# jibanCat/gp_dla_detection

Hardware: NVIDIA B200
Metric: qso_spectra_per_sec_10k_dla_samples (higher is better)
Workload: dtype f64

## Files before the change

### gp_dla_detection_b200/_lib.py

```python
from __future__ import annotations

import ctypes
import os

HERE = os.path.dirname(os.path.abspath(__file__))
LIB_PATH = os.environ.get("GPDLA_LIB", os.path.join(HERE, "libgpdla.so"))

c_double_p = ctypes.POINTER(ctypes.c_double)
c_u8_p = ctypes.POINTER(ctypes.c_uint8)
c_i32_p = ctypes.POINTER(ctypes.c_int32)
c_i64_p = ctypes.POINTER(ctypes.c_int64)

GPDLA_OK, GPDLA_ERR_INVALID, GPDLA_ERR_CUDA, GPDLA_ERR_UNSUPPORTED, GPDLA_ERR_STATE = 0, 1, 2, 3, 4
MAX_LINES = 31


class GpdlaParams(ctypes.Structure):
    _fields_ = [("min_lambda", ctypes.c_double), ("max_lambda", ctypes.c_double),
                ("lya_wavelength", ctypes.c_double), ("lyman_limit", ctypes.c_double),
                ("prior_z_qso_increase", ctypes.c_double), ("min_z_cut", ctypes.c_double),
                ("max_z_cut", ctypes.c_double), ("pixel_spacing", ctypes.c_double),
                ("num_lines", ctypes.c_int32), ("batch_quasars", ctypes.c_int32),
                ("gram_digits", ctypes.c_int32), ("rest_table", ctypes.c_int32)]

# ... 19 lines not shown
                       "log_posteriors_no_dla", "log_posteriors_lls", "log_posteriors_dla", "model_posteriors",
                       "p_no_dlas", "p_lls", "p_dlas", "MAP_z_dlas", "MAP_log_nhis", "MAP_inds",
                       "sample_log_likelihoods_dla", "sample_log_likelihoods_lls", "base_sample_inds"]


class GpdlaMultiResults(ctypes.Structure):
    _fields_ = [(n, ctypes.c_void_p) for n in MULTI_RESULT_FIELDS]


RECONSTRUCTION_FIELDS = ["absorption", "prior_mean", "prior_sd", "fit_mean", "continuum", "continuum_sd", "latent", "chi2",
                         "log_likelihood", "num_pixels"]


class GpdlaReconstruction(ctypes.Structure):
    _fields_ = [(n, ctypes.c_void_p) for n in RECONSTRUCTION_FIELDS]


SYMBOLS = {
    "gpdla_default_parameters": (None, [ctypes.POINTER(GpdlaParams)]),
    "gpdla_create": (ctypes.c_int, [ctypes.POINTER(ctypes.c_void_p), ctypes.c_int]),
    "gpdla_destroy": (None, [ctypes.c_void_p]),
    "gpdla_last_error": (ctypes.c_char_p, [ctypes.c_void_p]),
    "gpdla_launch_count": (ctypes.c_uint64, [ctypes.c_void_p]),
    "gpdla_set_profiling": (ctypes.c_int, [ctypes.c_void_p, ctypes.c_int]),
    "gpdla_profile_read": (ctypes.c_int, [ctypes.c_void_p, ctypes.POINTER(ctypes.c_double), c_i64_p]),
    "gpdla_set_parameters": (ctypes.c_int, [ctypes.c_void_p, ctypes.POINTER(GpdlaParams)]),
    "gpdla_set_model": (ctypes.c_int, [ctypes.c_void_p, c_double_p, ctypes.c_int32, c_double_p, c_double_p,
                                       ctypes.c_int32, c_double_p, ctypes.c_double, ctypes.c_double,
                                       ctypes.c_double]),
    "gpdla_set_samples": (ctypes.c_int, [ctypes.c_void_p, c_double_p, c_double_p, c_double_p, ctypes.c_int64]),
    "gpdla_set_prior": (ctypes.c_int, [ctypes.c_void_p, c_double_p, c_u8_p, ctypes.c_int64]),
    "gpdla_process_qsos": (ctypes.c_int, [ctypes.c_void_p, ctypes.c_int64, ctypes.c_int64, ctypes.c_void_p,
                                          ctypes.c_void_p, ctypes.c_void_p, ctypes.c_void_p, ctypes.c_void_p,
                                          ctypes.c_void_p, ctypes.POINTER(GpdlaResults)]),
    "gpdla_process_qsos_device": (ctypes.c_int, [ctypes.c_void_p, ctypes.c_int64, ctypes.c_int64, ctypes.c_void_p,
                                                 ctypes.c_void_p, ctypes.c_void_p, ctypes.c_void_p,
                                                 ctypes.c_void_p, ctypes.c_void_p, ctypes.POINTER(GpdlaResults),
                                                 ctypes.c_void_p]),
    "gpdla_set_lls_samples": (ctypes.c_int, [ctypes.c_void_p, c_double_p, ctypes.c_int64, ctypes.c_double,
                                             ctypes.c_double]),
    "gpdla_process_qsos_multi": (ctypes.c_int, [ctypes.c_void_p, ctypes.c_int64, ctypes.c_int64] + [ctypes.c_void_p] * 6
                                 + [ctypes.c_int32, ctypes.c_void_p, ctypes.POINTER(GpdlaMultiResults)]),
    "gpdla_process_qsos_multi_device": (ctypes.c_int, [ctypes.c_void_p, ctypes.c_int64, ctypes.c_int64]
                                        + [ctypes.c_void_p] * 6 + [ctypes.c_int32, ctypes.c_void_p,
                                                                   ctypes.POINTER(GpdlaMultiResults), ctypes.c_void_p]),
    "gpdla_matlab_default_rand": (None, [c_double_p, ctypes.c_int64]),
    "gpdla_voigt": (ctypes.c_int, [c_double_p, ctypes.c_int64, ctypes.c_double, ctypes.c_double, ctypes.c_int32,
                                   c_double_p]),
    "gpdla_voigt_batch_device": (ctypes.c_int, [ctypes.c_void_p, ctypes.c_int64, ctypes.c_void_p, ctypes.c_void_p,
                                                ctypes.c_int64, ctypes.c_int32, ctypes.c_void_p, ctypes.c_void_p]),
    "gpdla_line_constants": (None, [c_double_p, c_double_p, c_double_p, c_double_p]),
    "gpdla_rest_table": (ctypes.c_int, [ctypes.c_int32, ctypes.c_double, c_double_p, c_i32_p, c_i32_p, c_double_p,
                                        c_double_p]),
    "gpdla_host_alloc": (ctypes.c_int, [ctypes.POINTER(ctypes.c_void_p), ctypes.c_uint64]),
    "gpdla_host_free": (None, [ctypes.c_void_p]),
    "gpdla_objective": (ctypes.c_int, [ctypes.c_int64, ctypes.c_int32, ctypes.c_int32] + [ctypes.c_void_p] * 6),
    "gpdla_objective_device": (ctypes.c_int, [ctypes.c_int64, ctypes.c_int32, ctypes.c_int32] + [ctypes.c_void_p] * 7),
    "gpdla_objective_lyseries": (ctypes.c_int, [ctypes.c_int64, ctypes.c_int32, ctypes.c_int32] + [ctypes.c_void_p] * 3
                                 + [ctypes.c_int32, c_double_p, c_double_p] + [ctypes.c_void_p] * 3),
    "gpdla_objective_lyseries_device": (ctypes.c_int, [ctypes.c_int64, ctypes.c_int32, ctypes.c_int32] + [ctypes.c_void_p] * 3
                                        + [ctypes.c_int32, c_double_p, c_double_p] + [ctypes.c_void_p] * 4),
    "gpdla_default_preload_parameters": (None, [ctypes.POINTER(GpdlaPreloadParams)]),
    "gpdla_preload_qsos": (ctypes.c_int, [ctypes.c_int64, ctypes.c_int64] + [ctypes.c_void_p] * 7
                           + [ctypes.POINTER(GpdlaPreloadParams), ctypes.c_int64] + [ctypes.c_void_p] * 7),
    "gpdla_preload_qsos_device": (ctypes.c_int, [ctypes.c_int64, ctypes.c_int64] + [ctypes.c_void_p] * 7
                                  + [ctypes.POINTER(GpdlaPreloadParams), ctypes.c_int64] + [ctypes.c_void_p] * 8),
    "gpdla_training_set": (ctypes.c_int, [ctypes.c_int64, ctypes.c_int64] + [ctypes.c_void_p] * 7
                           + [ctypes.c_int32, ctypes.c_double, ctypes.c_double] + [ctypes.c_void_p] * 6),
    "gpdla_training_set_device": (ctypes.c_int, [ctypes.c_int64, ctypes.c_int64] + [ctypes.c_void_p] * 7
                                  + [ctypes.c_int32, ctypes.c_double, ctypes.c_double] + [ctypes.c_void_p] * 7),
    "gpdla_pairwise_covariance": (ctypes.c_int, [ctypes.c_int64, ctypes.c_int32] + [ctypes.c_void_p] * 3),
    "gpdla_pairwise_covariance_device": (ctypes.c_int, [ctypes.c_int64, ctypes.c_int32] + [ctypes.c_void_p] * 4),
    "gpdla_training_set_lyseries": (ctypes.c_int, [ctypes.c_int64, ctypes.c_int64] + [ctypes.c_void_p] * 7
                                    + [ctypes.c_int32, ctypes.c_double, ctypes.c_double, ctypes.c_int32]
                                    + [ctypes.c_void_p] * 7),
    "gpdla_training_set_lyseries_device": (ctypes.c_int, [ctypes.c_int64, ctypes.c_int64] + [ctypes.c_void_p] * 7
                                           + [ctypes.c_int32, ctypes.c_double, ctypes.c_double, ctypes.c_int32]
                                           + [ctypes.c_void_p] * 8),
    "gpdla_row_nanmedian_fill": (ctypes.c_int, [ctypes.c_int64, ctypes.c_int32] + [ctypes.c_void_p] * 2),
    "gpdla_row_nanmedian_fill_device": (ctypes.c_int, [ctypes.c_int64, ctypes.c_int32] + [ctypes.c_void_p] * 3),
    "gpdla_dla_statistics": (ctypes.c_int, [ctypes.c_int64, ctypes.c_int64] + [ctypes.c_void_p] * 8
                             + [ctypes.c_int32, c_double_p, ctypes.c_int32, c_double_p, ctypes.c_double, ctypes.c_double,
                                ctypes.c_void_p]),
    "gpdla_dla_statistics_device": (ctypes.c_int, [ctypes.c_int64, ctypes.c_int64] + [ctypes.c_void_p] * 8
                                    + [ctypes.c_int32, c_double_p, ctypes.c_int32, c_double_p, ctypes.c_double,
                                       ctypes.c_double, ctypes.c_void_p, ctypes.c_void_p]),
    "gpdla_multi_dla_statistics": (ctypes.c_int, [ctypes.c_int64, ctypes.c_int64, ctypes.c_int32] + [ctypes.c_void_p] * 9
                                   + [ctypes.c_int32, c_double_p, ctypes.c_int32, c_double_p, ctypes.c_double,
                                      ctypes.c_double, ctypes.c_void_p]),
    "gpdla_multi_dla_statistics_device": (ctypes.c_int, [ctypes.c_int64, ctypes.c_int64, ctypes.c_int32]
                                          + [ctypes.c_void_p] * 9
                                          + [ctypes.c_int32, c_double_p, ctypes.c_int32, c_double_p, ctypes.c_double,
                                             ctypes.c_double, ctypes.c_void_p, ctypes.c_void_p]),
    "gpdla_reconstruct": (ctypes.c_int, [ctypes.c_void_p, ctypes.c_int64, ctypes.c_int64] + [ctypes.c_void_p] * 6
                          + [ctypes.c_int32, ctypes.c_int32, ctypes.c_void_p, ctypes.c_void_p,
                             ctypes.POINTER(GpdlaReconstruction)]),
    "gpdla_reconstruct_device": (ctypes.c_int, [ctypes.c_void_p, ctypes.c_int64, ctypes.c_int64] + [ctypes.c_void_p] * 6
                                 + [ctypes.c_int32, ctypes.c_int32, ctypes.c_void_p, ctypes.c_void_p,
                                    ctypes.POINTER(GpdlaReconstruction), ctypes.c_void_p]),
}

_lib = None


def load() -> ctypes.CDLL:
    global _lib
# ... 24 lines not shown
```

### gp_dla_detection_b200/csrc/gpdla_capi.cu

```cuda
#include <cuda_runtime.h>
#include <math.h>
#include <stdio.h>
#include <stdlib.h>
#include <string.h>

#include <algorithm>
#include <cmath>
#include <map>
#include <mutex>
#include <numeric>
#include <random>
#include <string>
#include <vector>

#include "../../include/gpdla.h"
#include "gpdla_kernels.cuh"
#include "gpdla_i8_kernels.cuh"
#include "gpdla_preload.cuh"
#include "gpdla_objective.cuh"
#include "gpdla_training.cuh"
#include "gpdla_statistics.cuh"
#include "gpdla_reconstruct.cuh"
#include "gpdla_rest_table.h"

// ... 273 lines not shown
  int mws_batch = 0, mws_npix = 0;
  int64_t mws_S = 0;
  double *d_acache = nullptr, *d_msll = nullptr, *d_mlls = nullptr, *d_cum = nullptr, *d_mscal = nullptr;
  int32_t *d_partners = nullptr, *d_active = nullptr;
  bool profiling = false;
  std::vector<std::pair<cudaEvent_t, cudaEvent_t>> prof_events;
};

static int i8_digits(const gpdla_ctx* c) {
  int d = c->params.gram_digits;
  if (d == 0) d = 6;
  if (c->k == I8_K_EXT && (d == 5 || d == 6)) return 6;
  return (c->k == I8_K && (d == 5 || d == 6)) ? d : 0;
}
static int64_t gram_rows(const gpdla_ctx* c) { return ((int64_t)c->S + 1 + i8::TM - 1) / i8::TM * i8::TM; }
static bool use_i8(const gpdla_ctx* c) { return i8_digits(c) > 0; }

static void free_workspace(gpdla_ctx* c) {
  cudaFree(c->d_meta); cudaFree(c->d_lam); cudaFree(c->d_lamh); cudaFree(c->d_pix); cudaFree(c->d_Mq); cudaFree(c->d_P);
  cudaFree(c->d_sll); cudaFree(c->d_scratch); cudaFree(c->d_scratch_i); cudaFree(c->d_gram); cudaFree(c->d_qld);
  c->d_gram = c->d_qld = nullptr;
  c->d_meta = nullptr; c->d_lam = c->d_lamh = c->d_pix = c->d_Mq = c->d_P = c->d_sll = c->d_scratch = nullptr;
  c->d_scratch_i = nullptr;
  c->ws_batch = c->ws_npix = c->ws_k = 0; c->ws_S = 0;
}

static int ensure_workspace(gpdla_ctx* c, int batch, int npix) {
  if (c->ws_batch >= batch && c->ws_npix == npix && c->ws_k == c->k && c->ws_S == c->S) return GPDLA_OK;
  free_workspace(c);
  const size_t B = batch;
  CUDA_TRY(cudaMalloc(&c->d_meta, B * sizeof(QuasarMeta)), c->err);
  CUDA_TRY(cudaMalloc(&c->d_lam, B * (npix + 8) * sizeof(double)), c->err);
  CUDA_TRY(cudaMalloc(&c->d_lamh, B * (npix + 8) * sizeof(double)), c->err);
  CUDA_TRY(cudaMalloc(&c->d_pix, B * npix * 4 * sizeof(double)), c->err);
  CUDA_TRY(cudaMalloc(&c->d_Mq, B * npix * c->k * sizeof(double)), c->err);
  CUDA_TRY(cudaMalloc(&c->d_P, B * (npix / KC) * gram_doubles_per_chunk_all_splits(c->k) * sizeof(double)), c->err);
  CUDA_TRY(cudaMalloc(&c->d_sll, B * c->S * sizeof(double)), c->err);
  CUDA_TRY(cudaMalloc(&c->d_scratch, B * 16 * sizeof(double)), c->err);
  CUDA_TRY(cudaMalloc(&c->d_scratch_i, B * sizeof(int64_t)), c->err);
  if (rank_splits(c->k) > 1) {
    const size_t rows = (size_t)gram_rows(c);
    CUDA_TRY(cudaMalloc(&c->d_gram, B * rows * rank_ncol(c->k) * sizeof(double)), c->err);
    CUDA_TRY(cudaMalloc(&c->d_qld, B * rows * 2 * sizeof(double)), c->err);
  }
  c->ws_batch = batch; c->ws_npix = npix; c->ws_k = c->k; c->ws_S = c->S;
  return GPDLA_OK;
}

static int ensure_rest_table(gpdla_ctx* c) {
  if (c->params.rest_table < 0) return GPDLA_OK;
  if (c->d_rt && c->rt_num_lines == c->params.num_lines && c->rt_pixel_spacing == c->params.pixel_spacing) return GPDLA_OK;
  LineConstants lc;
  fill_line_constants(&lc);
  const RestTableHost t = build_rest_table(c->params.num_lines, c->params.pixel_spacing, RT_NEAR_PIXELS, lc.tw, lc.lc,
                                           lc.gam, kSigma, kC);
  std::vector<double> cells((size_t)RT_PLANES * t.ncell * 2, 0.0);
  for (int p = 0; p <= RT_DEG_DEV; ++p)
    for (int ci = 0; ci < t.ncell; ++ci) cells[((size_t)(p / 2) * t.ncell + ci) * 2 + (p & 1)] = t.coef[(size_t)p * t.ncell + ci];
  int rc = dev_upload(&c->d_rt, cells.data(), cells.size(), c->err);
  if (rc) return rc;
  c->rt_ncell = t.ncell; c->rt_h = t.h; c->rt_num_lines = c->params.num_lines; c->rt_pixel_spacing = c->params.pixel_spacing;
  return GPDLA_OK;
}
static RestTable rest_table_args(const gpdla_ctx* c) {
  RestTable rt;
  const bool on = c->params.rest_table >= 0 && c->d_rt != nullptr;
  rt.coef = on ? c->d_rt : nullptr;
  rt.ncell = c->rt_ncell;
  rt.inv_h = 1.0 / (c->params.pixel_spacing * log(10.0));
  rt.lam_lo = RT_LAMBDA_LO;
  return rt;
}

constexpr int FALLBACK_SLOTS = 8;
template <int K, int NL, int MODE, int NSPLIT>
static int launch_loglik(gpdla_ctx* c, LoglikArgs la, int nq, cudaStream_t st, bool timed = true) {
  using WCfg = WsConfig<K, NSPLIT>;
  auto kern = dla_loglik_ws_kernel<K, NL, MODE, NSPLIT>;
  if (la.only_list) {
    if constexpr (K == I8_K || K == I8_K_EXT) kern = dla_loglik_ws_list_kernel<K, NL, MODE, NSPLIT>;
    else { c->err = "FP64 fallback list: rank without an INT8 path"; return GPDLA_ERR_UNSUPPORTED; }
  }
  const size_t smem = WCfg::smem_bytes(la.num_lines);
  const int TS = WCfg::TS;
  int rc = configure_smem(c->device, kern, smem, c->err);
  if (rc) return rc;
  const unsigned tiles = (unsigned)((la.S + (la.log_likelihoods_no_dla ? 1 : 0) + TS - 1) / TS);
  dim3 grid(tiles, la.only_list ? (unsigned)std::min(nq, FALLBACK_SLOTS) : (unsigned)nq, NSPLIT);
  la.gram = c->d_gram; la.qld = c->d_qld; la.gram_rows = gram_rows(c);
  cudaEvent_t e0 = nullptr, e1 = nullptr;
  if (c->profiling && timed) {
    CUDA_TRY(cudaEventCreate(&e0), c->err);
    CUDA_TRY(cudaEventCreate(&e1), c->err);
    CUDA_TRY(cudaEventRecord(e0, st), c->err);
  }
  kern<<<grid, WS_THREADS, smem, st>>>(la);
  c->launches++;
  CUDA_TRY(cudaGetLastError(), c->err);
  if (NSPLIT > 1 && !la.only_list) {
    CholArgs ca;
    ca.meta = la.meta; ca.gram = c->d_gram; ca.qld = c->d_qld; ca.gram_rows = la.gram_rows; ca.S = la.S;
    ca.sample_log_likelihoods = la.sample_log_likelihoods; ca.sll_stride = la.sll_stride;
    ca.log_likelihoods_no_dla = la.log_likelihoods_no_dla; ca.active = la.active; ca.order = la.order;
    ca.q_offset = la.q_offset;
    rc = configure_smem(c->device, cholesky_kernel<K>, cholesky_smem_bytes<K>(), c->err);
    if (rc) return rc;
    cholesky_kernel<K><<<dim3(tiles * TS / CHOL_SAMPLES, (unsigned)nq), CHOL_THREADS,
                         cholesky_smem_bytes<K>(), st>>>(ca);
    c->launches++;
    CUDA_TRY(cudaGetLastError(), c->err);
  }
// ... 290 lines not shown
  int rc = launch_mode_i8<MODE>(c, la, nq - nq_f64, st);
  if (rc == GPDLA_OK) {
    CUDA_TRY(cudaStreamWaitEvent(c->side_stream, c->ev_fork, 0), c->err);
    LoglikArgs lf = la;
    lf.q_offset = nq - nq_f64;
    rc = launch_mode<MODE>(c, lf, nq_f64, c->side_stream, false);
    CUDA_TRY(cudaEventRecord(c->ev_join, c->side_stream), c->err);
    CUDA_TRY(cudaStreamWaitEvent(st, c->ev_join, 0), c->err);
  }
  if (timed) {
    c->profiling = true;
    CUDA_TRY(cudaEventRecord(e1, st), c->err);
    c->prof_events.emplace_back(e0, e1);
  }
  return rc;
}

__global__ void fill_i32_kernel(int32_t* p, int32_t v, int64_t n) {
  int64_t i = (int64_t)blockIdx.x * blockDim.x + threadIdx.x;
  if (i < n) p[i] = v;
}

extern "C" {

void gpdla_default_parameters(gpdla_params* p) {
  const double c = 299792458.0;
  p->min_lambda = 911.75; p->max_lambda = 1215.75;
  p->lya_wavelength = 1215.6701; p->lyman_limit = 911.7633;
  p->prior_z_qso_increase = (30000.0 * 1000.0) / c;
  p->min_z_cut = (3000.0 * 1000.0) / c; p->max_z_cut = (3000.0 * 1000.0) / c;
  p->pixel_spacing = 1e-4;
  p->num_lines = 3;
  p->batch_quasars = 0;
  p->gram_digits = 0; p->rest_table = 0;
}

int gpdla_rest_table(int32_t num_lines, double pixel_spacing, double* coef, int32_t* ncell, int32_t* degree, double* h,
                     double* lambda_lo) {
  if (num_lines < 1 || num_lines > GPDLA_MAX_LINES || !(pixel_spacing > 0)) return GPDLA_ERR_INVALID;
  LineConstants lc;
  fill_line_constants(&lc);
  if (degree) *degree = RT_DEG;
  if (lambda_lo) *lambda_lo = RT_LAMBDA_LO;
  if (!coef) {
    const double hh = pixel_spacing * log(10.0);
    if (h) *h = hh;
    if (ncell) *ncell = (int32_t)ceil((log(RT_LAMBDA_HI) - log(RT_LAMBDA_LO)) / hh) + 1;
    return GPDLA_OK;
  }
  const RestTableHost t = build_rest_table(num_lines, pixel_spacing, RT_NEAR_PIXELS, lc.tw, lc.lc, lc.gam, kSigma, kC);
  memcpy(coef, t.coef.data(), t.coef.size() * sizeof(double));
  if (ncell) *ncell = t.ncell;
  if (h) *h = t.h;
  return GPDLA_OK;
}

int gpdla_host_alloc(void** ptr, uint64_t bytes) {
  if (!ptr) return GPDLA_ERR_INVALID;
  *ptr = nullptr;
  CUDA_TRY(cudaHostAlloc(ptr, bytes > 0 ? bytes : 1, cudaHostAllocDefault), g_err);
  return GPDLA_OK;
}
void gpdla_host_free(void* ptr) { if (ptr) cudaFreeHost(ptr); }

void gpdla_line_constants(double* tw, double* lcs, double* gam, double* ip) {
  LineConstants lc;
  fill_line_constants(&lc);
  if (tw) memcpy(tw, lc.tw, sizeof lc.tw);
  if (lcs) memcpy(lcs, lc.lc, sizeof lc.lc);
  if (gam) memcpy(gam, lc.gam, sizeof lc.gam);
  if (ip) memcpy(ip, lc.ip, sizeof lc.ip);
}

int gpdla_create(gpdla_ctx** out, int device) {
  if (!out) return GPDLA_ERR_INVALID;
  *out = nullptr;
  int ndev = 0;
  if (cudaGetDeviceCount(&ndev) != cudaSuccess || device < 0 || device >= ndev || device >= MAX_DEVICES) {
    g_err = "no CUDA device " + std::to_string(device) + " (libgpdla.so has no CPU fallback)";
    return GPDLA_ERR_CUDA;
  }
  DeviceGuard guard(device);
  if (guard.status != cudaSuccess) { g_err = cudaGetErrorString(guard.status); return GPDLA_ERR_CUDA; }
  int rc = upload_device_constants(g_err);
  if (rc != GPDLA_OK) return rc;
  gpdla_ctx* ctx = new gpdla_ctx;
  ctx->device = device;
  gpdla_default_parameters(&ctx->params);
  cudaError_t e = cudaStreamCreateWithFlags(&ctx->stream, cudaStreamNonBlocking);
  if (e == cudaSuccess) e = cudaStreamCreateWithFlags(&ctx->copy_stream, cudaStreamNonBlocking);
  if (e == cudaSuccess) e = cudaStreamCreateWithFlags(&ctx->side_stream, cudaStreamNonBlocking);
  if (e == cudaSuccess) e = cudaEventCreateWithFlags(&ctx->ev_fork, cudaEventDisableTiming);
  if (e == cudaSuccess) e = cudaEventCreateWithFlags(&ctx->ev_join, cudaEventDisableTiming);
  for (int i = 0; i < 2 && e == cudaSuccess; ++i) {
    e = cudaEventCreateWithFlags(&ctx->ev_batch[i], cudaEventDisableTiming);
    if (e == cudaSuccess) e = cudaEventCreateWithFlags(&ctx->ev_copied[i], cudaEventDisableTiming);
  }
  if (e != cudaSuccess) { g_err = cudaGetErrorString(e); gpdla_destroy(ctx); return GPDLA_ERR_CUDA; }
  *out = ctx;
  return GPDLA_OK;
}

void gpdla_destroy(gpdla_ctx* c) {
  if (!c) return;
  DeviceGuard guard(c->device);
  if (c->stream) cudaStreamSynchronize(c->stream);
// ... 1419 lines not shown
```

### gp_dla_detection_b200/csrc/gpdla_i8_kernels.cuh

```cuda
#pragma once
#include "gpdla_kernels.cuh"

namespace gpdla {
namespace i8 {

constexpr int CLUSTER = 4;
constexpr int TS = 32;
constexpr int TM = CLUSTER * TS;
constexpr int WCTAS = 3;
constexpr int NPROD = 8;
constexpr int SPB = TS / NPROD;
constexpr int NCTRL = 4;
constexpr int THREADS = 32 * (NCTRL + NPROD);
constexpr int STAGES = 3;
constexpr double CAP = 0.996;
constexpr int TMEM_COLS = 512;
#ifndef GPDLA_I8P_PROBE
#define GPDLA_I8P_PROBE 0
#endif
constexpr int PROBE = GPDLA_I8P_PROBE;
#ifndef GPDLA_I8P_SHFL_CONV
#define GPDLA_I8P_SHFL_CONV 0
#endif
#ifndef GPDLA_I8P_PF
// ... 781 lines not shown
        }
      }
      __syncwarp();
      if (!Sh::EXT && lane == 0) mbar_arrive(&bar_sq[it & 1]);
      if (GPDLA_I8P_PHASES && xa.phase && lane == 0) {
        atomicAdd(&xa.phase[8 + 1], (unsigned long long)w_empty); atomicAdd(&xa.phase[8 + 14], (unsigned long long)w_hand);
        w_empty = w_hand = 0;
        if (pr == 0) atomicAdd(&xa.phase[7], 1ull);
      }
      ++it;
    }
  } else if (warp >= NCTRL) {
    asm volatile("setmaxnreg.inc.sync.aligned.u32 %0;" ::"n"(REG_A));
    const int pr = warp - NCTRL;
    const int row0 = pr * SPB;
    double* myraw = rawbuf + row0 * RAWS;
    double* hb = hbuf + pr * (2 * SPB * KC) + lane;
    uint64_t* const hfull = bar_hfull + 2 * pr;
    uint64_t* const hempty = bar_hempty + 2 * pr;
    uint32_t gh = 0;
    long long w_hand = 0;
    for (int t = cluster_id; t < num_tiles; t += num_clusters) {
      const int q = tile_quasar(t);
      const QuasarMeta meta = args.meta[q];
      if (!tile_live(q, meta)) continue;
      const int64_t s0 = (int64_t)(t % tiles_per_quasar) * TM + (int64_t)rank * TS;
      const int nchunks = meta.nchunks;
      __syncwarp();
      if (lane < SPB) {
        const int i = row0 + lane;
        const int64_t s = s0 + i;
        const bool is_null = s >= S;
        const int64_t so = sample_at(args, is_null ? S - 1 : s);
        const double z = __dadd_rn(meta.min_z_dla, __dmul_rn(meta.max_z_dla - meta.min_z_dla, args.offset_samples[so]));
        s_nhi[i] = is_null ? -1.0 : args.nhi_samples[so];
        s_K[i] = rest_table_offset(args.rt, z, meta.lam_ref);
        s_so[i] = (int)so;
        for (int j = 0; j < num_lines; ++j) s_mult[j * TS + i] = line_multiplier(j, z);
        if (MODE == 2) {
          for (int j = 0; j < args.num_partners; ++j)
            s_part[j * TS + i] = is_null ? 0 : args.partners[((int64_t)q * 3 + j) * S + so];
        }
      }
      __syncwarp();
      const double* lam = args.lam_pad + (int64_t)q * (args.NPIX + 8);
      const double2* pix8 = reinterpret_cast<const double2*>(xa.pix8 + (int64_t)q * args.NPIX * 8);
      double* const cache_q = (MODE != 0) ? args.acache + (int64_t)q * S * args.NPIX : nullptr;

      const double* lamh = args.lamh + (int64_t)q * (args.NPIX + 8);
      double K_mid;
      const int tab_mode = (MODE != 2) ? group_cell<SPB>(args.rt, s_K + row0, K_mid) : 0;
      auto eval_raw = [&](double lambda, double lh, double (&e)[SPB], const RestCell* cell = nullptr) {
        double tau[SPB];
        tau_samples<NL, SPB>(args.rt, tab_mode, K_mid, lambda, lh, s_mult + row0, TS, s_K + row0, num_lines, tau, cell);
        raw_from_tau<SPB, false>(tau, s_nhi + row0, e);
      };
      double eprev[SPB];
      if (MODE != 2) {
        double e[SPB];
        eval_raw(lam[lane < 6 ? lane : 5], lamh[lane < 6 ? lane : 5], e);
        if (CONV_B) {
          const uint32_t slot = gh & 1u;
          mbar_wait_d(&hempty[slot], ((gh >> 1) & 1u) ^ 1u, xa.status, 15);
#pragma unroll
          for (int ss = NCA; ss < SPB; ++ss) hb[(slot * SPB + ss) * KC] = e[ss];
          __syncwarp();
          if (lane == 0) mbar_arrive(&hfull[slot]);
          ++gh;
        }
        if (SHFL_CONV) {
#pragma unroll
          for (int ss = 0; ss < SPB; ++ss) eprev[ss] = __shfl_sync(0xffffffffu, e[ss], (lane + 6) & 31);
        } else if (lane < 6) {
#pragma unroll
          for (int ss = 0; ss < NCA; ++ss) myraw[ss * RAWS + lane] = e[ss];
        }
      }
      double rows_n[4][SPB];
      auto load_rows = [&](int ipix) {
#pragma unroll
        for (int ss = 0; ss < SPB; ++ss) rows_n[0][ss] = cache_q[(int64_t)s_so[row0 + ss] * args.NPIX + ipix];
#pragma unroll
        for (int j = 0; j < 3; ++j)
          if (j < args.num_partners) {
#pragma unroll
            for (int ss = 0; ss < SPB; ++ss) rows_n[1 + j][ss] = cache_q[(int64_t)s_part[j * TS + row0 + ss] * args.NPIX + ipix];
          }
      };
      if (MODE == 2) load_rows(lane);
      const double2* prec = pix8 + lane;
      double2 plln = prec[0];
      double2 plln2 = prec[nchunks > 1 ? KC : 0];
      RestCell cell_n;
      const bool use_cell = GPDLA_I8P_PF && MODE != 2 && tab_mode == 1;
      if (use_cell) rest_table_fetch(args.rt, plln.y, K_mid, cell_n);
      for (int c = 0; c < nchunks; ++c) {
        const int i = c * KC + lane;
        const double lambda = plln.x, lh = plln.y;
        const RestCell cell = cell_n;
        plln = plln2;
        if (c + 2 < nchunks) {
          prec += KC;
          plln2 = prec[KC];
        }
        if (use_cell && c + 1 < nchunks) rest_table_fetch(args.rt, plln.y, K_mid, cell_n);
        double a[SPB];
        if (MODE != 2) {
// ... 157 lines not shown
```

### gp_dla_detection_b200/csrc/gpdla_kernels.cuh

```cuda
#pragma once
#include <stdint.h>
#include "gpdla_math.cuh"

namespace gpdla {

constexpr int KC = 32;
constexpr int RAWW = 64;
constexpr int NTHREADS = 256;
constexpr double LOG_2PI = 1.83787706640934534;

struct QuasarMeta {
  int n_u;
  int n;
  int nchunks;
  int first;
  double min_z_dla, max_z_dla;
  double log_prior_no_dla, log_prior_dla;
  int prior_num_quasars, prior_num_dlas;
  double lam_ref;
};

struct ForestConstants {
  double wavelength[MAX_LINES];
  double tau_ratio[MAX_LINES];
// ... 480 lines not shown
struct TauRow { double t[SPB]; };

template <int NL, int SPB>
__device__ __noinline__ TauRow<SPB> tau_direct(double lambda, const double* mymult, int mstride, int num_lines) {
  TauRow<SPB> out;
  double (&tau)[SPB] = out.t;
  if (NL == 3) {
    const int lane = threadIdx.x & 31;
    unsigned cm[SPB], any = 0;
#pragma unroll
    for (int ss = 0; ss < SPB; ++ss) {
      bool core;
      tau[ss] = tau_sum_3_wing(lambda, mymult[ss], mymult[mstride + ss], mymult[2 * mstride + ss], core);
      cm[ss] = __ballot_sync(0xffffffffu, core);
      any |= cm[ss];
    }
    if (any) {
      int off[SPB + 1];
      off[0] = 0;
#pragma unroll
      for (int ss = 0; ss < SPB; ++ss) off[ss + 1] = off[ss] + __popc(cm[ss]);
      if (off[SPB] <= 32) {
        int ss_i = 0;
#pragma unroll
        for (int ss = 1; ss < SPB; ++ss) ss_i = (lane >= off[ss]) ? ss : ss_i;
        unsigned mask_i = cm[0];
        int off_i = 0;
#pragma unroll
        for (int ss = 1; ss < SPB; ++ss) { mask_i = (ss_i == ss) ? cm[ss] : mask_i; off_i = (ss_i == ss) ? off[ss] : off_i; }
        const bool have = lane < off[SPB];
        const int src = have ? (int)__fns(mask_i, 0, lane - off_i + 1) : 0;
        const double lam_i = __shfl_sync(0xffffffffu, lambda, src);
        const double t = tau_sum_3_exact(lam_i, mymult[ss_i], mymult[mstride + ss_i], mymult[2 * mstride + ss_i]);
        const unsigned below = (1u << lane) - 1u;
#pragma unroll
        for (int ss = 0; ss < SPB; ++ss) {
          const double v = __shfl_sync(0xffffffffu, t, (off[ss] + __popc(cm[ss] & below)) & 31);
          if ((cm[ss] >> lane) & 1u) tau[ss] = v;
        }
      } else {
#pragma unroll
        for (int ss = 0; ss < SPB; ++ss)
          if ((cm[ss] >> lane) & 1u)
            tau[ss] = tau_sum_3_exact(lambda, mymult[ss], mymult[mstride + ss], mymult[2 * mstride + ss]);
      }
    }
  } else {
#pragma unroll
    for (int ss = 0; ss < SPB; ++ss) tau[ss] = tau_sum_generic(lambda, mymult + ss, mstride, num_lines);
  }
  return out;
}

template <int SPB>
__device__ __forceinline__ bool tau_from_cell(const RestCell& rc, const double* myK, double (&tau)[SPB]) {
  unsigned worst = 0;
#pragma unroll
  for (int ss = 0; ss < SPB; ++ss) {
    tau[ss] = rest_table_eval(rc, myK[ss]);
    worst = max(worst, (unsigned)__double2hiint(tau[ss]));
  }
  return __any_sync(0xffffffffu, worst >= 0x7ff00000u);
}

template <int SPB>
__device__ __noinline__ TauRow<SPB> tau_own_cells(const RestTable& rt, double lh, const double* myK) {
  TauRow<SPB> out;
#pragma unroll
  for (int ss = 0; ss < SPB; ++ss) {
    RestCell rc;
    const double K = myK[ss];
    rest_table_fetch(rt, lh, K, rc);
    out.t[ss] = rest_table_eval(rc, K);
  }
  return out;
}

template <int NL, int SPB>
__device__ __forceinline__ void tau_samples(const RestTable& rt, int tab_mode, double K_mid, double lambda, double lh,
                                            const double* mymult, int mstride, const double* myK, int num_lines,
                                            double (&tau)[SPB], const RestCell* cell = nullptr) {
  bool direct = tab_mode == 0;
  if (tab_mode == 1) {
    RestCell rc;
    if (cell) rc = *cell;
    else rest_table_fetch(rt, lh, K_mid, rc);
    direct = tau_from_cell<SPB>(rc, myK, tau);
  } else if (tab_mode == 2) {
    const TauRow<SPB> r = tau_own_cells<SPB>(rt, lh, myK);
    unsigned worst = 0;
#pragma unroll
    for (int ss = 0; ss < SPB; ++ss) { tau[ss] = r.t[ss]; worst = max(worst, (unsigned)__double2hiint(tau[ss])); }
    direct = __any_sync(0xffffffffu, worst >= 0x7ff00000u);
  }
  if (direct) {
    const TauRow<SPB> r = tau_direct<NL, SPB>(lambda, mymult, mstride, num_lines);
#pragma unroll
    for (int ss = 0; ss < SPB; ++ss) tau[ss] = r.t[ss];
  }
}

template <int SPB, bool EXP_TABLE = (GPDLA_EXP_TABLE != 0)>
__device__ __forceinline__ void raw_from_tau(const double (&tau)[SPB], const double* mynhi, double (&e)[SPB]) {
#pragma unroll
  for (int ss = 0; ss < SPB; ++ss) e[ss] = -mynhi[ss] * tau[ss];
#pragma unroll
  for (int ss = 0; ss < SPB; ++ss) e[ss] = exp_nonpos<EXP_TABLE>(e[ss]);
}

template <int SPB>
__device__ __forceinline__ int group_cell(const RestTable& rt, const double* myK, double& K_mid) {
  double lo = myK[0], hi = myK[0];
#pragma unroll
  for (int ss = 1; ss < SPB; ++ss) { lo = fmin(lo, myK[ss]); hi = fmax(hi, myK[ss]); }
  K_mid = 0.5 * (lo + hi);
  return rt.coef == nullptr ? 0 : ((hi - lo) <= RT_MAX_SPREAD ? 1 : 2);
}

template <int K, int NSPLIT>
struct WsConfig {
  using G = GramShape<K>;
  using SS = SplitShape<K, NSPLIT>;
  static constexpr int SPW = 8;
  static constexpr int SPB = 4;
  static constexpr int TS = WS_CONSUMERS * SPW;
  static constexpr int SPP = TS / WS_PRODUCERS;
  static constexpr size_t B_BYTES = 2ull * SS::CHUNK_DOUBLES * 8;
  static constexpr size_t A_BYTES = (size_t)WS_STAGES * 2 * TS * ASTR * 8;
  static constexpr size_t RAW_BYTES = (size_t)TS * RAWS * 8;
  static constexpr int CSTR = TS + 4;
  static constexpr size_t C_BYTES = (size_t)((K + 1) * (K + 2) / 2) * CSTR * 8;
  static_assert(NSPLIT > 1 || C_BYTES <= B_BYTES + A_BYTES, "epilogue staging must fit");
  static_assert(SS::NTL * 4 + 40 <= 168, "accumulators must fit in the consumer's registers");
  static constexpr int NBAR = 2 + 2 * WS_STAGES * WS_CONSUMERS;
  __host__ __device__ static constexpr size_t smem_bytes(int num_lines) {
    return B_BYTES + A_BYTES + RAW_BYTES + (size_t)TS * (num_lines + 4) * 8 + NBAR * 8 + 64 + 4 * TS * 4;
  }
};

__device__ __forceinline__ void mbar_inval(uint64_t* bar) {
  asm volatile("mbarrier.inval.shared::cta.b64 [%0];" ::"r"(smem_u32(bar)) : "memory");
}

template <int K, int NL, int MODE, int NSPLIT>
__device__ __forceinline__ void ws_tile(const LoglikArgs& args, const int q) {
  using Cfg = WsConfig<K, NSPLIT>;
  using G = GramShape<K>;
  using SS = SplitShape<K, NSPLIT>;
  constexpr int TS = Cfg::TS, SPW = Cfg::SPW, SPB = Cfg::SPB, SPP = Cfg::SPP, NT = SS::NTL, CSTR = Cfg::CSTR;
// ... 28 lines not shown
  uint64_t* bar_full = bar_p + 2;
  uint64_t* bar_empty = bar_full + WS_STAGES * WS_CONSUMERS;
  int* s_done = reinterpret_cast<int*>(bar_empty + WS_STAGES * WS_CONSUMERS);
  int* s_part = s_done + 2;
  int* s_so = s_part + 3 * TS;
  double* Cs = reinterpret_cast<double*>(smem_raw);

  for (int i = tid; i < TS; i += WS_THREADS) {
    const int64_t s = s0 + i;
    const bool is_null = s >= S;
    const int64_t so = sample_at(args, is_null ? S - 1 : s);
    const double z = __dadd_rn(meta.min_z_dla, __dmul_rn(meta.max_z_dla - meta.min_z_dla, args.offset_samples[so]));
    s_nhi[i] = is_null ? -1.0 : args.nhi_samples[so];
    s_ld[i] = 0.0;
    s_K[i] = rest_table_offset(args.rt, z, meta.lam_ref);
    s_so[i] = (int)so;
    for (int j = 0; j < num_lines; ++j) s_mult[j * TS + i] = line_multiplier(j, z);
    if (MODE == 2) {
      for (int j = 0; j < args.num_partners; ++j)
        s_part[j * TS + i] = is_null ? 0 : args.partners[((int64_t)q * 3 + j) * S + so];
    }
  }
  const double* Pq = args.P + ((int64_t)q * NSPLIT + split) * (args.NPIX / KC) * SS::CHUNK_DOUBLES;
  constexpr uint32_t CHUNK_BYTES = SS::CHUNK_DOUBLES * 8;
  if (tid == 0) {
    mbar_init(&bar_p[0], 1);
    mbar_init(&bar_p[1], 1);
    for (int i = 0; i < WS_STAGES * WS_CONSUMERS; ++i) { mbar_init(&bar_full[i], 64); mbar_init(&bar_empty[i], 32); }
    s_done[0] = 0; s_done[1] = 0;
    asm volatile("fence.mbarrier_init.release.cluster;" ::: "memory");
    mbar_expect_tx(&bar_p[0], CHUNK_BYTES);
    tma_load_1d(Bt, Pq, CHUNK_BYTES, &bar_p[0]);
    if (meta.nchunks > 1) {
      mbar_expect_tx(&bar_p[1], CHUNK_BYTES);
      tma_load_1d(Bt + SS::CHUNK_DOUBLES, Pq + SS::CHUNK_DOUBLES, CHUNK_BYTES, &bar_p[1]);
    }
  }
  __syncthreads();

  double acc[NT][2];

  if (warp >= WS_CONSUMERS) {
    const int pr = warp - WS_CONSUMERS;
    const double* lam = args.lam_pad + (int64_t)q * (args.NPIX + 8);
    const double* pix = args.pix + (int64_t)q * args.NPIX * 4;
    double* const cache_q = (MODE != 0) ? args.acache + (int64_t)q * S * args.NPIX : nullptr;
    auto batch_consumer = [&](int b) { return (pr + b * WS_PRODUCERS) % WS_CONSUMERS; };
    auto batch_row0 = [&](int b) { return batch_consumer(b) * SPW + ((pr + b * WS_PRODUCERS) / WS_CONSUMERS) * SPB; };

    const double* lamh = args.lamh + (int64_t)q * (args.NPIX + 8);
    auto eval_raw = [&](int row0, double lambda, double lh, double (&e)[SPB]) {
      double tau[SPB], K_mid;
      const int tab_mode = group_cell<SPB>(args.rt, s_K + row0, K_mid);
      tau_samples<NL, SPB>(args.rt, tab_mode, K_mid, lambda, lh, s_mult + row0, TS, s_K + row0, num_lines, tau);
      raw_from_tau<SPB>(tau, s_nhi + row0, e);
    };
    if (MODE != 2) {
      const double lambda0 = lam[lane < 6 ? lane : 5], lh0 = lamh[lane < 6 ? lane : 5];
#pragma unroll
      for (int b = 0; b < SPP / SPB; ++b) {
        double e[SPB];
        eval_raw(batch_row0(b), lambda0, lh0, e);
        if (lane < 6) {
#pragma unroll
          for (int ss = 0; ss < SPB; ++ss) rawbuf[(batch_row0(b) + ss) * RAWS + lane] = e[ss];
        }
      }
    }
    double qacc[SPP], ldm[SPP];
    int lde[SPP];
#pragma unroll
    for (int ss = 0; ss < SPP; ++ss) { qacc[ss] = 0.0; ldm[ss] = 1.0; lde[ss] = 0; }

    double lambda_n = lam[6 + lane], lh_n = lamh[6 + lane];
    double2 p01n = *reinterpret_cast<const double2*>(pix + (int64_t)lane * 4);
    double2 p23n = *reinterpret_cast<const double2*>(pix + (int64_t)lane * 4 + 2);
    for (int c = 0; c < meta.nchunks; ++c) {
      const int stage = c % WS_STAGES;
      const int i = c * KC + lane;
      const double lambda = lambda_n, lh = lh_n;
      const double y = p01n.x, v = p01n.y, mu = p23n.x, om2 = p23n.y;
      if (c + 1 < meta.nchunks) {
        lambda_n = lam[i + KC + 6];
        lh_n = lamh[i + KC + 6];
        p01n = *reinterpret_cast<const double2*>(pix + (int64_t)(i + KC) * 4);
        p23n = *reinterpret_cast<const double2*>(pix + (int64_t)(i + KC) * 4 + 2);
      }
#pragma unroll
      for (int b = 0; b < SPP / SPB; ++b) {
        const int cons = batch_consumer(b), row0 = batch_row0(b);
        double* myraw = rawbuf + row0 * RAWS;
        double a[SPB];
        if (MODE != 2) {
          double e[SPB];
          eval_raw(row0, lambda, lh, e);
#pragma unroll
          for (int ss = 0; ss < SPB; ++ss) myraw[ss * RAWS + 6 + lane] = e[ss];
          __syncwarp();
          double carry[SPB];
#pragma unroll
          for (int ss = 0; ss < SPB; ++ss) {
            const double* rb = myraw + ss * RAWS;
            double acc_a = 0.0;
#pragma unroll
            for (int t = 0; t < 6; ++t) acc_a = fma(rb[lane + t], c_lines.ip[t], acc_a);
            acc_a = fma(e[ss], c_lines.ip[6], acc_a);
            carry[ss] = rb[KC + (lane < 6 ? lane : 0)];
// ... 519 lines not shown
```

### gp_dla_detection_b200/csrc/gpdla_rest_table.h

```cpp
#pragma once
#include <math.h>

#include <complex>
#include <vector>

namespace gpdla {

constexpr int RT_DEG = 8;
constexpr double RT_HALF_WIDTH = 1.0;
constexpr double RT_LAMBDA_LO = 880.0;
constexpr double RT_LAMBDA_HI = 1720.0;
constexpr double RT_NEAR_PIXELS = 16.0;

struct RestTableHost {
  std::vector<double> coef;
  int ncell = 0;
  double h = 0;
  double ln_lo = 0;
};

inline long double rest_table_tau(long double x , int num_lines, const double* tw,
                                  const double* lc, const double* gam, double sigma, double c) {
  const long double s2 = sqrtl(2.0L) * (long double)sigma;
  long double total = 0.0L;
  for (int j = 0; j < num_lines; ++j) {
    const long double v = (long double)c * expm1l(x - logl((long double)tw[j] * 1e8L));
    const std::complex<long double> z(v / s2, (long double)gam[j] / s2);
    const std::complex<long double> iz2 = 1.0L / (2.0L * z * z);
    std::complex<long double> term(1.0L, 0.0L), sum(1.0L, 0.0L);
    for (int n = 1; n < 40; ++n) {
      term *= (long double)(2 * n - 1) * iz2;
      sum += term;
      if (std::abs(term) < 1e-22L) break;
    }
    const std::complex<long double> w = std::complex<long double>(0.0L, 1.0L) / (sqrtl(M_PIl) * z) * sum;
    total += (long double)lc[j] * w.real() / (sqrtl(2.0L * M_PIl) * (long double)sigma);
  }
  return total;
}

inline RestTableHost build_rest_table(int num_lines, double pixel_spacing_dex, double near_pixels, const double* tw,
                                      const double* lc, const double* gam, double sigma, double c) {
  RestTableHost t;
  t.h = pixel_spacing_dex * log(10.0);
  t.ln_lo = log(RT_LAMBDA_LO);
  t.ncell = (int)ceil((log(RT_LAMBDA_HI) - t.ln_lo) / t.h) + 1;
  constexpr int n = RT_DEG + 1;
  t.coef.assign((size_t)n * t.ncell, 0.0);
  long double nodes[n], Tm[n][n] = {};
  for (int k = 0; k < n; ++k) nodes[k] = cosl(M_PIl * (k + 0.5L) / n);
  Tm[0][0] = 1.0L;
  Tm[1][1] = 1.0L;
  for (int j = 2; j < n; ++j)
    for (int p = 0; p < n; ++p) Tm[j][p] = (p > 0 ? 2.0L * Tm[j - 1][p - 1] : 0.0L) - Tm[j - 2][p];
  std::vector<double> centre(num_lines);
  for (int j = 0; j < num_lines; ++j) centre[j] = (log(tw[j] * 1e8) - t.ln_lo) / t.h;
  for (int cidx = 0; cidx < t.ncell; ++cidx) {
    bool near = (cidx == 0 || cidx == t.ncell - 1);
    for (int j = 0; j < num_lines; ++j) near |= fabs((double)cidx - centre[j]) < near_pixels + 0.5;
    if (near) {
      for (int p = 0; p < n; ++p) t.coef[(size_t)p * t.ncell + cidx] = NAN;
      continue;
    }
    long double f[n], cj[n];
    for (int k = 0; k < n; ++k)
      f[k] = rest_table_tau((long double)t.ln_lo + (long double)t.h * ((long double)cidx + (long double)RT_HALF_WIDTH * nodes[k]),
                            num_lines, tw, lc, gam, sigma, c);
    for (int j = 0; j < n; ++j) {
      long double a = 0.0L;
      for (int k = 0; k < n; ++k) a += f[k] * cosl(M_PIl * j * (k + 0.5L) / n);
      cj[j] = a * (j == 0 ? 1.0L : 2.0L) / n;
    }
    long double scale = 1.0L;
    for (int p = 0; p < n; ++p) {
      long double m = 0.0L;
      for (int j = 0; j < n; ++j) m += cj[j] * Tm[j][p];
      t.coef[(size_t)p * t.ncell + cidx] = (double)(m * scale);
      scale /= (long double)RT_HALF_WIDTH;
    }
  }
  return t;
}

}
```

### include/gpdla.h

```cpp
#ifndef GPDLA_H
#define GPDLA_H

#include <stdint.h>

#ifdef __cplusplus
extern "C" {
#endif

#define GPDLA_OK 0
#define GPDLA_ERR_INVALID 1
#define GPDLA_ERR_CUDA 2
#define GPDLA_ERR_UNSUPPORTED 3
#define GPDLA_ERR_STATE 4

#define GPDLA_MAX_LINES 31

typedef struct gpdla_ctx gpdla_ctx;

typedef struct {
  double min_lambda;
  double max_lambda;
  double lya_wavelength;
  double lyman_limit;
  double prior_z_qso_increase;
// ... 156 lines not shown
int gpdla_dla_statistics(int64_t Q, int64_t S, const double* sample_log_likelihoods_dla, const double* p_dlas,
                         const double* min_z_dlas, const double* max_z_dlas, const uint8_t* select,
                         const double* offset_samples, const double* log_nhi_samples, const double* nhi_samples,
                         int32_t n_z, const double* z_edges, int32_t n_nhi, const double* log_nhi_edges,
                         double dla_log_nhi_min, double omega_m, double* sums);
int gpdla_dla_statistics_device(int64_t Q, int64_t S, const double* sample_log_likelihoods_dla, const double* p_dlas,
                                const double* min_z_dlas, const double* max_z_dlas, const uint8_t* select,
                                const double* offset_samples, const double* log_nhi_samples, const double* nhi_samples,
                                int32_t n_z, const double* z_edges, int32_t n_nhi, const double* log_nhi_edges,
                                double dla_log_nhi_min, double omega_m, double* sums, void* stream);

int gpdla_multi_dla_statistics(int64_t Q, int64_t S, int32_t max_dlas, const double* sample_log_likelihoods_dla,
                               const int32_t* base_sample_inds, const double* model_posteriors,
                               const double* min_z_dlas, const double* max_z_dlas, const uint8_t* select,
                               const double* offset_samples, const double* log_nhi_samples, const double* nhi_samples,
                               int32_t n_z, const double* z_edges, int32_t n_nhi, const double* log_nhi_edges,
                               double dla_log_nhi_min, double omega_m, double* sums);
int gpdla_multi_dla_statistics_device(int64_t Q, int64_t S, int32_t max_dlas, const double* sample_log_likelihoods_dla,
                                      const int32_t* base_sample_inds, const double* model_posteriors,
                                      const double* min_z_dlas, const double* max_z_dlas, const uint8_t* select,
                                      const double* offset_samples, const double* log_nhi_samples,
                                      const double* nhi_samples, int32_t n_z, const double* z_edges, int32_t n_nhi,
                                      const double* log_nhi_edges, double dla_log_nhi_min, double omega_m,
                                      double* sums, void* stream);

typedef struct {
  double* absorption;
  double* prior_mean;
  double* prior_sd;
  double* fit_mean;
  double* continuum;
  double* continuum_sd;
  double* latent;
  double* chi2;
  double* log_likelihood;
  int32_t* num_pixels;
} gpdla_reconstruction;
int gpdla_reconstruct(gpdla_ctx* ctx, int64_t Q, int64_t L_max, const double* wavelengths, const double* flux,
                      const double* noise_variance, const uint8_t* pixel_mask, const int32_t* lengths,
                      const double* z_qsos, int32_t meanflux, int32_t num_absorbers, const double* absorber_z,
                      const double* absorber_nhi, const gpdla_reconstruction* out);
int gpdla_reconstruct_device(gpdla_ctx* ctx, int64_t Q, int64_t L_max, const double* wavelengths, const double* flux,
                             const double* noise_variance, const uint8_t* pixel_mask, const int32_t* lengths,
                             const double* z_qsos, int32_t meanflux, int32_t num_absorbers, const double* absorber_z,
                             const double* absorber_nhi, const gpdla_reconstruction* out, void* stream);

int gpdla_voigt(const double* lambdas, int64_t num_points, double z, double N, int32_t num_lines, double* profile);
int gpdla_voigt_batch_device(const double* lambdas, int64_t num_points, const double* z, const double* N,
                             int64_t S, int32_t num_lines, double* profile, void* stream);

int gpdla_rest_table(int32_t num_lines, double pixel_spacing, double* coef, int32_t* ncell, int32_t* degree,
                     double* h, double* lambda_lo);

int gpdla_host_alloc(void** ptr, uint64_t bytes);
void gpdla_host_free(void* ptr);

void gpdla_line_constants(double* transition_wavelengths, double* leading_constants, double* gammas,
                          double* instrument_profile);

#ifdef __cplusplus
}
#endif
#endif
```

Baseline: 5697.

## Tabulate other-line remainder near single Lyman line and evaluate nearest line directly

Rest-frame tau table cells near exactly one line (for 3-line runs) no longer store NaN. They hold the Chebyshev fit of the other lines' contribution and are tagged by negating the coefficients. On the device, a new fixup routine adds the nearest line's wing or core profile to the tabulated remainder, packing core evaluations across the warp with ballots and shuffles, instead of falling back to full direct evaluation of all lines. The goal is fewer costly direct-tau fallbacks near line centres, at the price of more complex warp-level code and a new sign-tag convention in the table.

```diff
diff --git a/gp_dla_detection_b200/_lib.py b/gp_dla_detection_b200/_lib.py
--- a/gp_dla_detection_b200/_lib.py
+++ b/gp_dla_detection_b200/_lib.py
@@ -95,6 +95,7 @@
     "gpdla_line_constants": (None, [c_double_p, c_double_p, c_double_p, c_double_p]),
     "gpdla_rest_table": (ctypes.c_int, [ctypes.c_int32, ctypes.c_double, c_double_p, c_i32_p, c_i32_p, c_double_p,
                                         c_double_p]),
+    "gpdla_rest_table_tagged": (ctypes.c_int, [ctypes.c_int32, ctypes.c_double, c_double_p, c_i32_p]),
     "gpdla_host_alloc": (ctypes.c_int, [ctypes.POINTER(ctypes.c_void_p), ctypes.c_uint64]),
     "gpdla_host_free": (None, [ctypes.c_void_p]),
     "gpdla_objective": (ctypes.c_int, [ctypes.c_int64, ctypes.c_int32, ctypes.c_int32] + [ctypes.c_void_p] * 6),
diff --git a/gp_dla_detection_b200/csrc/gpdla_capi.cu b/gp_dla_detection_b200/csrc/gpdla_capi.cu
--- a/gp_dla_detection_b200/csrc/gpdla_capi.cu
+++ b/gp_dla_detection_b200/csrc/gpdla_capi.cu
@@ -349,11 +349,25 @@
   if (c->d_rt && c->rt_num_lines == c->params.num_lines && c->rt_pixel_spacing == c->params.pixel_spacing) return GPDLA_OK;
   LineConstants lc;
   fill_line_constants(&lc);
+  std::vector<int> tag;
   const RestTableHost t = build_rest_table(c->params.num_lines, c->params.pixel_spacing, RT_NEAR_PIXELS, lc.tw, lc.lc,
-                                           lc.gam, kSigma, kC);
+                                           lc.gam, kSigma, kC, &tag);
   std::vector<double> cells((size_t)RT_PLANES * t.ncell * 2, 0.0);
   for (int p = 0; p <= RT_DEG_DEV; ++p)
-    for (int ci = 0; ci < t.ncell; ++ci) cells[((size_t)(p / 2) * t.ncell + ci) * 2 + (p & 1)] = t.coef[(size_t)p * t.ncell + ci];
+    for (int ci = 0; ci < t.ncell; ++ci)
+      cells[((size_t)(p / 2) * t.ncell + ci) * 2 + (p & 1)] = tag[ci] ? -t.coef[(size_t)p * t.ncell + ci] : t.coef[(size_t)p * t.ncell + ci];
+#if GPDLA_I8P_PROBE & 128
+  auto plain = [&](int ci) { return !std::isnan(t.coef[ci]) && tag[ci] == 0; };
+  for (int ci = 0; ci < t.ncell; ++ci) {
+    if (plain(ci)) continue;
+    int best = -1;
+    for (int d = 1; best < 0 && d < t.ncell; ++d) {
+      if (ci - d >= 0 && plain(ci - d)) best = ci - d;
+      else if (ci + d < t.ncell && plain(ci + d)) best = ci + d;
+    }
+    for (int p = 0; p <= RT_DEG_DEV; ++p) cells[((size_t)(p / 2) * t.ncell + ci) * 2 + (p & 1)] = p == 0 ? t.coef[best] : 0.0;
+  }
+#endif
   int rc = dev_upload(&c->d_rt, cells.data(), cells.size(), c->err);
   if (rc) return rc;
   c->rt_ncell = t.ncell; c->rt_h = t.h; c->rt_num_lines = c->params.num_lines; c->rt_pixel_spacing = c->params.pixel_spacing;
@@ -750,6 +764,17 @@
   memcpy(coef, t.coef.data(), t.coef.size() * sizeof(double));
   if (ncell) *ncell = t.ncell;
   if (h) *h = t.h;
+  return GPDLA_OK;
+}
+
+int gpdla_rest_table_tagged(int32_t num_lines, double pixel_spacing, double* coef, int32_t* tag) {
+  if (num_lines < 1 || num_lines > GPDLA_MAX_LINES || !(pixel_spacing > 0) || !coef || !tag) return GPDLA_ERR_INVALID;
+  LineConstants lc;
+  fill_line_constants(&lc);
+  std::vector<int> tg;
+  const RestTableHost t = build_rest_table(num_lines, pixel_spacing, RT_NEAR_PIXELS, lc.tw, lc.lc, lc.gam, kSigma, kC, &tg);
+  memcpy(coef, t.coef.data(), t.coef.size() * sizeof(double));
+  for (int ci = 0; ci < t.ncell; ++ci) tag[ci] = tg[ci];
   return GPDLA_OK;
 }
 
diff --git a/gp_dla_detection_b200/csrc/gpdla_i8_kernels.cuh b/gp_dla_detection_b200/csrc/gpdla_i8_kernels.cuh
--- a/gp_dla_detection_b200/csrc/gpdla_i8_kernels.cuh
+++ b/gp_dla_detection_b200/csrc/gpdla_i8_kernels.cuh
@@ -857,7 +857,7 @@
       const int tab_mode = (MODE != 2) ? group_cell<SPB>(args.rt, s_K + row0, K_mid) : 0;
       auto eval_raw = [&](double lambda, double lh, double (&e)[SPB], const RestCell* cell = nullptr) {
         double tau[SPB];
-        tau_samples<NL, SPB>(args.rt, tab_mode, K_mid, lambda, lh, s_mult + row0, TS, s_K + row0, num_lines, tau, cell);
+        tau_samples<NL, SPB, false>(args.rt, tab_mode, K_mid, lambda, lh, s_mult + row0, TS, s_K + row0, num_lines, tau, cell);
         raw_from_tau<SPB, false>(tau, s_nhi + row0, e);
       };
       double eprev[SPB];
diff --git a/gp_dla_detection_b200/csrc/gpdla_kernels.cuh b/gp_dla_detection_b200/csrc/gpdla_kernels.cuh
--- a/gp_dla_detection_b200/csrc/gpdla_kernels.cuh
+++ b/gp_dla_detection_b200/csrc/gpdla_kernels.cuh
@@ -556,6 +556,86 @@
   return out;
 }
 
+template <int NL, int SPB, bool KEEP_DIRECT>
+__device__ __noinline__ TauRow<SPB> tau_fixup(TauRow<SPB> tab, bool near_ok, double lambda, const double* mymult,
+                                              int mstride, int num_lines) {
+  if (NL == 3 && near_ok) {
+    unsigned nan = 0;
+#pragma unroll
+    for (int ss = 0; ss < SPB; ++ss) nan |= (((unsigned)__double2hiint(tab.t[ss]) & 0x7fffffffu) >= 0x7ff00000u);
+    if (!__any_sync(0xffffffffu, nan)) {
+      const int lane = threadIdx.x & 31;
+      const bool tagged = __double2hiint(tab.t[0]) < 0;
+      const double lim = c_wing3.v2min;
+      TauRow<SPB> rem, out;
+      unsigned cm[SPB], any = 0;
+      int j = 0;
+      {
+        const double v0 = fma(lambda, mymult[0], -c_lines.c), v1 = fma(lambda, mymult[mstride], -c_lines.c);
+        const double v2 = fma(lambda, mymult[2 * mstride], -c_lines.c);
+        const double s0 = v0 * v0, s1 = v1 * v1, s2 = v2 * v2;
+        j = hi_less(s1, s0) ? 1 : 0;
+        j = hi_less(s2, fmin(s0, s1)) ? 2 : j;
+      }
+#pragma unroll
+      for (int ss = 0; ss < SPB; ++ss) {
+        rem.t[ss] = -tab.t[ss];
+        double tj, sj;
+        if constexpr (KEEP_DIRECT) {
+          const double v0 = fma(lambda, mymult[ss], -c_lines.c), v1 = fma(lambda, mymult[mstride + ss], -c_lines.c);
+          const double v2 = fma(lambda, mymult[2 * mstride + ss], -c_lines.c);
+          const double s0 = v0 * v0, s1 = v1 * v1, s2 = v2 * v2;
+          const double t0 = tau_wing3_line(0, fast_rcp(s0)), t1 = tau_wing3_line(1, fast_rcp(s1));
+          const double t2 = tau_wing3_line(2, fast_rcp(s2));
+          tj = (j == 0) ? t0 : ((j == 1) ? t1 : t2);
+          sj = (j == 0) ? s0 : ((j == 1) ? s1 : s2);
+          out.t[ss] = tagged ? rem.t[ss] + tj : (t0 + t1) + t2;
+        } else {
+          const double v = fma(lambda, mymult[j * mstride + ss], -c_lines.c);
+          sj = v * v;
+          tj = tau_wing3_line(j, fast_rcp(sj));
+          out.t[ss] = tagged ? rem.t[ss] + tj : tab.t[ss];
+        }
+        cm[ss] = __ballot_sync(0xffffffffu, tagged && hi_less(sj, lim));
+        any |= cm[ss];
+      }
+      if (any) {
+        int off[SPB + 1];
+        off[0] = 0;
+#pragma unroll
+        for (int ss = 0; ss < SPB; ++ss) off[ss + 1] = off[ss] + __popc(cm[ss]);
+        if (off[SPB] <= 32) {
+          int ss_i = 0;
+#pragma unroll
+          for (int ss = 1; ss < SPB; ++ss) ss_i = (lane >= off[ss]) ? ss : ss_i;
+          unsigned mask_i = cm[0];
+          int off_i = 0;
+#pragma unroll
+          for (int ss = 1; ss < SPB; ++ss) { mask_i = (ss_i == ss) ? cm[ss] : mask_i; off_i = (ss_i == ss) ? off[ss] : off_i; }
+          const bool have = lane < off[SPB];
+          const int src = have ? (int)__fns(mask_i, 0, lane - off_i + 1) : 0;
+          const double lam_i = __shfl_sync(0xffffffffu, lambda, src);
+          const int j_i = __shfl_sync(0xffffffffu, j, src);
+          const double t = tau_core(j_i, __dsub_rn(__dmul_rn(lam_i, mymult[j_i * mstride + ss_i]), c_lines.c) * c_lines.inv_s2s);
+          const unsigned below = (1u << lane) - 1u;
+#pragma unroll
+          for (int ss = 0; ss < SPB; ++ss) {
+            const double v = __shfl_sync(0xffffffffu, t, (off[ss] + __popc(cm[ss] & below)) & 31);
+            if ((cm[ss] >> lane) & 1u) out.t[ss] = rem.t[ss] + v;
+          }
+        } else {
+#pragma unroll
+          for (int ss = 0; ss < SPB; ++ss)
+            if ((cm[ss] >> lane) & 1u)
+              out.t[ss] = rem.t[ss] + tau_core(j, __dsub_rn(__dmul_rn(lambda, mymult[j * mstride + ss]), c_lines.c) * c_lines.inv_s2s);
+        }
+      }
+      return out;
+    }
+  }
+  return tau_direct<NL, SPB>(lambda, mymult, mstride, num_lines);
+}
+
 template <int SPB>
 __device__ __forceinline__ bool tau_from_cell(const RestCell& rc, const double* myK, double (&tau)[SPB]) {
   unsigned worst = 0;
@@ -580,25 +660,28 @@
   return out;
 }
 
-template <int NL, int SPB>
+template <int NL, int SPB, bool KEEP_DIRECT>
 __device__ __forceinline__ void tau_samples(const RestTable& rt, int tab_mode, double K_mid, double lambda, double lh,
                                             const double* mymult, int mstride, const double* myK, int num_lines,
                                             double (&tau)[SPB], const RestCell* cell = nullptr) {
-  bool direct = tab_mode == 0;
+  bool rare = tab_mode == 0;
   if (tab_mode == 1) {
     RestCell rc;
     if (cell) rc = *cell;
     else rest_table_fetch(rt, lh, K_mid, rc);
-    direct = tau_from_cell<SPB>(rc, myK, tau);
+    rare = tau_from_cell<SPB>(rc, myK, tau);
   } else if (tab_mode == 2) {
     const TauRow<SPB> r = tau_own_cells<SPB>(rt, lh, myK);
     unsigned worst = 0;
 #pragma unroll
     for (int ss = 0; ss < SPB; ++ss) { tau[ss] = r.t[ss]; worst = max(worst, (unsigned)__double2hiint(tau[ss])); }
-    direct = __any_sync(0xffffffffu, worst >= 0x7ff00000u);
-  }
-  if (direct) {
-    const TauRow<SPB> r = tau_direct<NL, SPB>(lambda, mymult, mstride, num_lines);
+    rare = __any_sync(0xffffffffu, worst >= 0x7ff00000u);
+  }
+  if (rare) {
+    TauRow<SPB> r;
+#pragma unroll
+    for (int ss = 0; ss < SPB; ++ss) r.t[ss] = tau[ss];
+    r = tau_fixup<NL, SPB, KEEP_DIRECT>(r, tab_mode == 1, lambda, mymult, mstride, num_lines);
 #pragma unroll
     for (int ss = 0; ss < SPB; ++ss) tau[ss] = r.t[ss];
   }
@@ -733,7 +816,7 @@
     auto eval_raw = [&](int row0, double lambda, double lh, double (&e)[SPB]) {
       double tau[SPB], K_mid;
       const int tab_mode = group_cell<SPB>(args.rt, s_K + row0, K_mid);
-      tau_samples<NL, SPB>(args.rt, tab_mode, K_mid, lambda, lh, s_mult + row0, TS, s_K + row0, num_lines, tau);
+      tau_samples<NL, SPB, true>(args.rt, tab_mode, K_mid, lambda, lh, s_mult + row0, TS, s_K + row0, num_lines, tau);
       raw_from_tau<SPB>(tau, s_nhi + row0, e);
     };
     if (MODE != 2) {
diff --git a/gp_dla_detection_b200/csrc/gpdla_rest_table.h b/gp_dla_detection_b200/csrc/gpdla_rest_table.h
--- a/gp_dla_detection_b200/csrc/gpdla_rest_table.h
+++ b/gp_dla_detection_b200/csrc/gpdla_rest_table.h
@@ -20,10 +20,11 @@
 };
 
 inline long double rest_table_tau(long double x , int num_lines, const double* tw,
-                                  const double* lc, const double* gam, double sigma, double c) {
+                                  const double* lc, const double* gam, double sigma, double c, int skip = -1) {
   const long double s2 = sqrtl(2.0L) * (long double)sigma;
   long double total = 0.0L;
   for (int j = 0; j < num_lines; ++j) {
+    if (j == skip) continue;
     const long double v = (long double)c * expm1l(x - logl((long double)tw[j] * 1e8L));
     const std::complex<long double> z(v / s2, (long double)gam[j] / s2);
     const std::complex<long double> iz2 = 1.0L / (2.0L * z * z);
@@ -40,7 +41,8 @@
 }
 
 inline RestTableHost build_rest_table(int num_lines, double pixel_spacing_dex, double near_pixels, const double* tw,
-                                      const double* lc, const double* gam, double sigma, double c) {
+                                      const double* lc, const double* gam, double sigma, double c,
+                                      std::vector<int>* tag = nullptr) {
   RestTableHost t;
   t.h = pixel_spacing_dex * log(10.0);
   t.ln_lo = log(RT_LAMBDA_LO);
@@ -55,17 +57,22 @@
     for (int p = 0; p < n; ++p) Tm[j][p] = (p > 0 ? 2.0L * Tm[j - 1][p - 1] : 0.0L) - Tm[j - 2][p];
   std::vector<double> centre(num_lines);
   for (int j = 0; j < num_lines; ++j) centre[j] = (log(tw[j] * 1e8) - t.ln_lo) / t.h;
+  if (tag) tag->assign(t.ncell, 0);
   for (int cidx = 0; cidx < t.ncell; ++cidx) {
-    bool near = (cidx == 0 || cidx == t.ncell - 1);
-    for (int j = 0; j < num_lines; ++j) near |= fabs((double)cidx - centre[j]) < near_pixels + 0.5;
-    if (near) {
+    const bool end = (cidx == 0 || cidx == t.ncell - 1);
+    int nnear = 0, jnear = -1;
+    for (int j = 0; j < num_lines; ++j)
+      if (fabs((double)cidx - centre[j]) < near_pixels + 0.5) { ++nnear; jnear = j; }
+    const bool remainder = tag && num_lines == 3 && !end && nnear == 1;
+    if ((end || nnear > 0) && !remainder) {
       for (int p = 0; p < n; ++p) t.coef[(size_t)p * t.ncell + cidx] = NAN;
       continue;
     }
+    if (remainder) (*tag)[cidx] = jnear + 1;
     long double f[n], cj[n];
     for (int k = 0; k < n; ++k)
       f[k] = rest_table_tau((long double)t.ln_lo + (long double)t.h * ((long double)cidx + (long double)RT_HALF_WIDTH * nodes[k]),
-                            num_lines, tw, lc, gam, sigma, c);
+                            num_lines, tw, lc, gam, sigma, c, remainder ? jnear : -1);
     for (int j = 0; j < n; ++j) {
       long double a = 0.0L;
       for (int k = 0; k < n; ++k) a += f[k] * cosl(M_PIl * j * (k + 0.5L) / n);
diff --git a/include/gpdla.h b/include/gpdla.h
--- a/include/gpdla.h
+++ b/include/gpdla.h
@@ -232,6 +232,8 @@
 int gpdla_rest_table(int32_t num_lines, double pixel_spacing, double* coef, int32_t* ncell, int32_t* degree,
                      double* h, double* lambda_lo);
 
+int gpdla_rest_table_tagged(int32_t num_lines, double pixel_spacing, double* coef, int32_t* tag);
+
 int gpdla_host_alloc(void** ptr, uint64_t bytes);
 void gpdla_host_free(void* ptr);
 
```

New measurement: 5809 (median of 6 runs). 2.0% higher.
